# halismai/photobundle

Hardware: AMD Instinct MI355X
Metric: LM iters/sec + residuals/sec, 8-frame KITTI window, 50k pts, 5x5 patch (higher is better)
Workload: dtype f64; 1 GPU; configs[1]: 8-frame window, 50000 points/GPU, 5x5 patch, single level, dense visibility; image=1241x376 u8, observations=400000, sampler_precision=exact, channels=1, point_parameterisation=free world points (reference)

## Files before the change

### photobundle_amd/csrc/pba_batch.h

```cpp
#pragma once
#include "pba_kernels.h"

namespace pba {

constexpr int kMaxBatch = 64;
constexpr int kBatchSampleWaves = 4;

struct BatchWindow {
  SchurParams schur[2];
  ReduceSolveParams rsolve[2];
  SampleParams sample[2];
  const float* frames_mc;
  int32_t channels;
};

struct BatchLaunch {
  const BatchWindow* tab;
  int32_t n;
  int32_t begin[kMaxBatch + 1];
  uint8_t win[kMaxBatch];
  uint8_t mode[kMaxBatch];
  unsigned long long seq[kMaxBatch];
};

__device__ __forceinline__ int batch_entry(const BatchLaunch& L, const int b) {
  int lo = 0, hi = L.n;
  while (hi - lo > 1) {
    const int mid = (lo + hi) >> 1;
    if (L.begin[mid] <= b) lo = mid; else hi = mid;
  }
  return lo;
}

__global__ __launch_bounds__(kTile, 2) void k_schur_batch(const BatchLaunch L) {
  const int k = batch_entry(L, (int)blockIdx.x);
  const int b0 = L.begin[k], lb = (int)blockIdx.x - b0, lgrid = L.begin[k + 1] - b0;
  const int mode = L.mode[k];
  SchurParams p = L.tab[L.win[k]].schur[mode & 1];
  p.init_scale = (mode >> 1) & 1;
  p.pub_seq = L.seq[k] - 1;
  if (!schur_prologue(p, false, lb, (int)threadIdx.x)) return;
  __shared__ __attribute__((aligned(16))) char smem[kSchurSmemBytes];
  schur_body<const void>(p, smem, (int)threadIdx.x, lb, lgrid, nullptr, nullptr, true);
}

__global__ __launch_bounds__(kReduceThreads) void k_reduce_solve_batch(const BatchLaunch L) {
  extern __shared__ __attribute__((aligned(16))) char dyn_smem[];
  const int k = batch_entry(L, (int)blockIdx.x);
  const int b0 = L.begin[k], lb = (int)blockIdx.x - b0, lgrid = L.begin[k + 1] - b0;
  const int mode = L.mode[k];
  ReduceSolveParams rsp = L.tab[L.win[k]].rsolve[mode & 1];
  rsp.so.init_scale = (mode >> 1) & 1;
  if (mode & 1) rsp.fin.seq = L.seq[k];
  reduce_solve_wg(rsp, dyn_smem, lb, lgrid, (int)threadIdx.x);
}

template <int R, bool UNITW>
__global__ __launch_bounds__(kBatchSampleWaves * 64) __attribute__((amdgpu_waves_per_eu((R <= 2 ? PBA_SAMPLE_WAVES_PER_SIMD : (R >= 4 ? PBA_SAMPLE_WAVES_LARGE : 2)), (R <= 2 ? PBA_SAMPLE_WAVES_PER_SIMD : (R >= 4 ? PBA_SAMPLE_WAVES_LARGE : 2)))))
void k_sample_batch(const BatchLaunch L) {
  const int k = batch_entry(L, (int)blockIdx.x);
  const int b0 = L.begin[k], lb = (int)blockIdx.x - b0, lgrid = L.begin[k + 1] - b0;
  const int mode = L.mode[k];
  SampleParams p = L.tab[L.win[k]].sample[mode & 1];
  if (mode & 1) p.seq = L.seq[k];
  if (!sample_prologue<true>(p, false, lb, (int)threadIdx.x)) return;
  __shared__ SampleSmem<R, kBatchSampleWaves> sm;
  ResLane<R> unused;
  sample_wg<R, true, kBatchSampleWaves, true, UNITW, false, false, kMaxFrames, true>(p, sm, unused, xcd_logical_block(lb, lgrid), lgrid, (int)threadIdx.x);
}

template <int R, bool UNITW>
__global__ __launch_bounds__(kBatchSampleWaves * 64) __attribute__((amdgpu_waves_per_eu(PBA_MC_WAVES(R), PBA_MC_WAVES(R)))) void k_sample_mc_batch(const BatchLaunch L) {
  const int k = batch_entry(L, (int)blockIdx.x);
  const int b0 = L.begin[k], lb = (int)blockIdx.x - b0, lgrid = L.begin[k + 1] - b0;
  const int mode = L.mode[k];
  const BatchWindow& bw = L.tab[L.win[k]];
  SampleParams p = bw.sample[mode & 1];
  if (mode & 1) p.seq = L.seq[k];
  if (!sample_prologue<true>(p, false, lb, (int)threadIdx.x)) return;
  sample_mc_wg<R, true, kBatchSampleWaves, true, UNITW>(p, bw.frames_mc, bw.channels, lb, lgrid, (int)threadIdx.x);
}

}
```

### photobundle_amd/csrc/pba_kernels.h

```cpp
#pragma once
#include "pba_device.h"

#include <cfloat>
#include <climits>
#include <type_traits>

#ifndef PBA_PHASE_TIMING
#define PBA_PHASE_TIMING 0
#endif

#ifndef PBA_SAMPLE_WAVES_PER_SIMD
#define PBA_SAMPLE_WAVES_PER_SIMD 4
#endif
#ifndef PBA_SAMPLE_WAVES_LARGE
#define PBA_SAMPLE_WAVES_LARGE 2
#endif
#ifndef PBA_EXPERIMENT_SKIP_IRREGULAR
#define PBA_EXPERIMENT_SKIP_IRREGULAR 0
#endif
#ifndef PBA_WALK_ROWWISE
#define PBA_WALK_ROWWISE 0
#endif

#ifndef PBA_REC_SC1
// ... 469 lines not shown
  if (JAC) {
    sgx = 0.5f * vlerp_exact(dy, omdy, hlerp_exact(dx, omdx, tex_gx2(t11), tex_gx2(t12)), hlerp_exact(dx, omdx, tex_gx2(t21), tex_gx2(t22)));
    sgy = 0.5f * vlerp_exact(dy, omdy, hlerp_exact(dx, omdx, tex_gy2(t11), tex_gy2(t12)), hlerp_exact(dx, omdx, tex_gy2(t21), tex_gy2(t22)));
  }
}

__global__ void k_sample_probe(const uint32_t* __restrict__ frame, int rows, int cols, int n, const float* __restrict__ y,
                               const float* __restrict__ x, float* __restrict__ out) {
  const int i = blockIdx.x * blockDim.x + threadIdx.x;
  if (i >= n) return;
  float sI, sgx, sgy;
  sample_generic<true>(frame, rows, cols, y[i], x[i], sI, sgx, sgy);
  out[3 * i] = sI; out[3 * i + 1] = sgx; out[3 * i + 2] = sgy;
}

struct SampleParams {
  const uint32_t* frames;
  const CamGeom* geom;
  const double* xyz;
  const double* rays;
  const float* desc;
  const double* w2;
  const int32_t* obs_point;
  const uint8_t* obs_slot;
  double* rec;
  double* block_cost;
  int32_t* block_fail;
  int64_t rec_stride;
  int32_t n_obs, n_frames;
  int32_t rows, cols;
  double fx, fy, cx, cy;
  double huber;
  const int4* tile_info;
  const int2* lane_rec;
  const CamGeom* geom_prev;
  const double* xyz_prev;
  const double* rec_prev;
  const double* sp;
  const double* ptrec;
  const double* delta_c;
  double* block_bs;
  unsigned int* ticket;
  unsigned long long* stamp;
  double* scal;
  double* host_scal;
  unsigned long long* host_seq;
  unsigned long long seq;
  int32_t n_tiles;
  int32_t skip_backsub;
  LmState* lm;
  LmState* host_state;
  pba_iteration_summary* log;
  int32_t max_log;
  int32_t enq_cur;
  double* block_cost_alt;
  int32_t* block_fail_alt;
  int32_t decide;
  int32_t prec;
  double* xchg;
  int32_t xchg_rank, xchg_world;
  int32_t xchg_sys;
  unsigned long long* xchg_flag;
  unsigned long long xchg_seq;
  unsigned long long* dbg;
  LmState* lm_init_dst; const LmState* lm_init_src;
  unsigned long long* res_tag; unsigned res_epoch;
};

__device__ __forceinline__ void store_tagged(unsigned long long* w, unsigned ep, double v) {
  const unsigned long long e = (unsigned long long)ep << 32;
  __hip_atomic_store(w, e | (unsigned)__double2hiint(v), __ATOMIC_RELAXED, __HIP_MEMORY_SCOPE_AGENT);
  __hip_atomic_store(w + 1, e | (unsigned)__double2loint(v), __ATOMIC_RELAXED, __HIP_MEMORY_SCOPE_AGENT);
}
__device__ __forceinline__ bool load_tagged(const unsigned long long* w, unsigned ep, double& v) {
  const unsigned long long a = __hip_atomic_load(w, __ATOMIC_RELAXED, __HIP_MEMORY_SCOPE_AGENT);
  const unsigned long long b = __hip_atomic_load(w + 1, __ATOMIC_RELAXED, __HIP_MEMORY_SCOPE_AGENT);
  v = __hiloint2double((int)(unsigned)a, (int)(unsigned)b);
  return (unsigned)(a >> 32) == ep && (unsigned)(b >> 32) == ep;
}

constexpr int kBk = 26;
static_assert(kBk * sizeof(double) <= sizeof(CamGeom), "the compact table fits the second camera-table slot");

__device__ __forceinline__ bool fused_resolve_parity(SampleParams& p) {
  if (p.lm) {
    if (p.lm->done) return false;
    if (p.lm->cur != p.enq_cur) {
      const double* tx = p.xyz; p.xyz = p.xyz_prev; p.xyz_prev = tx;
      double* tr = p.rec; p.rec = const_cast<double*>(p.rec_prev); p.rec_prev = tr;
      const CamGeom* tg = p.geom; p.geom = p.geom_prev; p.geom_prev = tg;
      double* tc = p.block_cost; p.block_cost = p.block_cost_alt; p.block_cost_alt = tc;
      int32_t* tf = p.block_fail; p.block_fail = p.block_fail_alt; p.block_fail_alt = tf;
    }
  }
  return true;
}

template <bool FUSED>
__device__ __forceinline__ bool sample_prologue(SampleParams& p, const bool keep_dbg, const int bid, const int tix) {
  if (!keep_dbg) p.dbg = nullptr;
  if (FUSED && !fused_resolve_parity(p)) return false;
  if (FUSED && p.lm_init_dst && bid == 0 && tix < (int)(sizeof(LmState) / 4))
    reinterpret_cast<unsigned*>(p.lm_init_dst)[tix] = __hip_atomic_load(reinterpret_cast<const unsigned*>(p.lm_init_src) + tix, __ATOMIC_RELAXED, __HIP_MEMORY_SCOPE_SYSTEM);
  return true;
}

struct FusedIdx { int4 ti; int pt, slot, l0, cnt; };
template <int NT>
__device__ __forceinline__ FusedIdx fused_prefetch_indices(const SampleParams& p, int bid, const int tix) {
  FusedIdx f{make_int4(0, 0, 0, 0), 0, 0, 0, 0};
  const int tile = bid * (NT / 128) + (int)(tix >> 7);
  const int lt = tix & 127;
  if (tile < p.n_tiles) {
    f.ti = p.tile_info[tile];
    const int2 r = p.lane_rec[(size_t)tile * 128 + lt];
    f.pt = r.x;
    f.slot = r.y & 0xff; f.l0 = (r.y >> 8) & 0xff; f.cnt = (r.y >> 16) & 0xff;
  }
  return f;
}

template <int NT, bool AG = false>
__device__ __forceinline__ void fused_stage_step_table(const SampleParams& p, double* s_bk, const int tix) {
  if (!p.skip_backsub) {
    constexpr int GW = (int)(sizeof(CamGeom) / 8);
    constexpr int oT = (int)(offsetof(CamGeom, t) / 8), oR = (int)(offsetof(CamGeom, R) / 8), oD = (int)(offsetof(CamGeom, dR) / 8);
    constexpr int oF = (int)(offsetof(CamGeom, free_index) / 4);
    static_assert(offsetof(CamGeom, t) % 8 == 0 && offsetof(CamGeom, R) % 8 == 0 && offsetof(CamGeom, dR) % 8 == 0, "double words");
    const double* G = reinterpret_cast<const double*>(p.geom_prev);
    constexpr int IT = (kBk * kMaxFrames + NT - 1) / NT;
    const int n_e = kBk * p.n_frames;
#pragma unroll
    for (int u = 0; u < IT; ++u) {
      const int e_raw = tix + u * NT;
      const int e = e_raw < n_e ? e_raw : 0;
      const int a = e / kBk, k = e - a * kBk;
      const double* g = G + (size_t)a * GW;
      const double* dc = p.delta_c + 6 * a;
      const bool rot = (k >= 12) && (k < 21);
      const int j = rot ? k - 12 : 0;
      const int o0 = (k < 9) ? oR + k : ((k < 12) ? oT + (k - 9) : oD + j);
      auto ld = [](const double* q) { return AG ? load_agent(q) : *q; };
      const double w0 = ld(g + o0), w1 = ld(g + oD + 9 + j), w2 = ld(g + oD + 18 + j);
      const double d0 = ld(dc), d1 = ld(dc + 1), d2 = ld(dc + 2);
      const double dt = ld(dc + ((k >= 21 && k < 24) ? 3 + (k - 21) : 3));
      const int32_t fidx = AG ? __hip_atomic_load(reinterpret_cast<const int32_t*>(g) + oF, __ATOMIC_RELAXED, __HIP_MEMORY_SCOPE_AGENT)
                              : reinterpret_cast<const int32_t*>(g)[oF];
      double val = rot ? d0 * w0 + d1 * w1 + d2 * w2 : w0;
      if (k >= 21) val = (k < 24) ? dt : (double)fidx;
      if (e_raw < n_e) s_bk[e] = val;
    }
  }
}

template <int NT, class RL = const void>
__device__ __forceinline__ void fused_backsub(const SampleParams& p, const double* rays, const FusedIdx& fi, const double* s_bk,
                                              double* s_bs, int& pt, int& slot, int& obs, bool& active, double (&X)[3],
                                              double& bs_mcc, double& bs_st2, double& bs_x2, const int tix, RL* rl = nullptr) {
  constexpr bool RES = !std::is_void<RL>::value;
  const int half = tix >> 7, lt = tix & 127;
  const int4 ti = fi.ti;
  active = lt < ti.y;
  obs = ti.x + lt;
  int l0 = 0, cnt = 0;
  double c3[3] = {0.0, 0.0, 0.0};
  double pr[12], spk[3] = {1.0, 1.0, 1.0};
// ... 1166 lines not shown
    if (p.huber > 0.0 && cc > p.huber * p.huber) {
      const double r = sqrt(cc);
      rho0 = 2.0 * p.huber * r - p.huber * p.huber;
      rho1 = fmax(DBL_MIN, p.huber / r);
    }
    cost_obs = 0.5 * rho0;
    if (!isfinite(cc)) atomicOr(&s_fail, 1);
    if (JAC) {
      p.rec[0 * p.rec_stride + obs] = rho1 * m11;
      p.rec[1 * p.rec_stride + obs] = rho1 * m12;
      p.rec[2 * p.rec_stride + obs] = rho1 * m22;
      p.rec[3 * p.rec_stride + obs] = rho1 * b1;
      p.rec[4 * p.rec_stride + obs] = rho1 * b2;
      p.rec[5 * p.rec_stride + obs] = cost_obs;
    }
  }
  if (FUSED) {
    lds_barrier();
    fused_wave_step_sums(bs_mcc, bs_st2, bs_x2);
    fused_block_partials<WAVES>(p, bid, lane, wave, cost_obs, bs_mcc, bs_st2, bs_x2, s_red, s_fail, tix);
    fused_finalize<WAVES>(p, lane, wave, &s_base[0][0], reinterpret_cast<double*>(s_raw), 0ull, tix, n_blocks);
  } else {
    const double ws = wave_sum(cost_obs);
    if (lane == 0) s_red[wave] = ws;
    lds_barrier();
    if (tix == 0) {
      double a = 0.0;
#pragma unroll
      for (int w = 0; w < WAVES; ++w) a += s_red[w];
      p.block_cost[bid] = a;
      p.block_fail[bid] = s_fail;
    }
  }
}

template <int R, bool JAC, int WAVES, bool FUSED, bool UNITW, int MF = kMaxFrames>
__global__ __launch_bounds__(WAVES * 64) __attribute__((amdgpu_waves_per_eu(PBA_MC_WAVES(R), PBA_MC_WAVES(R)))) void k_sample_mc(SampleParams p_in, const float* __restrict__ frames_mc, int n_channels) {
  SampleParams p = p_in;
  if (!sample_prologue<FUSED>(p, false, (int)blockIdx.x, (int)threadIdx.x)) return;
  sample_mc_wg<R, JAC, WAVES, FUSED, UNITW, MF>(p, frames_mc, n_channels, (int)blockIdx.x, (int)gridDim.x, (int)threadIdx.x);
}

constexpr int kTile = 128;
constexpr int kObsStride = 37;

constexpr size_t kSchurSmemBytes = sizeof(double) * (kTile * kObsStride + kTile) + kTile * kMaxFrames;

struct SchurParams {
  const double* xyz;
  const double* rays;
  const CamGeom* geom;
  const double* rec;
  const int32_t* obs_point;
  const uint8_t* obs_slot;
  const int4* tile_info;
  const int2* lane_rec;
  double* sp;
  double* ptrec;
  double* partial;
  int64_t rec_stride;
  int32_t n_tiles, n_frames;
  int32_t n_free;
  int32_t n_pairs;
  int32_t part_stride;
  int32_t init_scale;
  int32_t jacobi;
  double fx, fy;
  double radius, inv_radius, min_diag, max_diag;
  unsigned long long* dbg;
  const LmState* lm;
  int32_t enq_cur;
  int32_t final_pass;
  const double* xyz_alt; const CamGeom* geom_alt; const double* rec_alt;
  LmState* pub_state; const double* pub_scal; double* pub_host_scal;
  unsigned long long* pub_host_seq; unsigned long long pub_seq;
  unsigned long long* stamp;
};

__device__ __forceinline__ int sym6(int i, int j) {
  const int a = i < j ? i : j, b = i < j ? j : i;
  return a * 6 - (a * (a - 1)) / 2 + (b - a);
}

template <class RL>
__device__ __forceinline__ void schur_body(SchurParams& p, char* smem, const int tid, const int part, const int n_parts, RL* rl,
                                           const CamGeom* geom_res, const bool has_tile) {
  constexpr bool RES = !std::is_void<RL>::value;
  double* s_obs = reinterpret_cast<double*>(smem);
  static_assert(1024 + kTile * 9 <= kTile * kObsStride && kMaxFrames * sizeof(CamGeom) <= 1024 * sizeof(double), "aliasing fits");
  double* s_vg = s_obs + 1024;
  double* s_tot = s_obs + 1024 + kTile * 9;
  uint16_t* s_ptl = reinterpret_cast<uint16_t*>(s_obs + 1024 + 2 * kTile * 9);
  static_assert(1024 + 2 * kTile * 9 + kTile / 4 <= kTile * kObsStride, "point totals fit before W | Y");
  double* s_red = s_obs + kTile * kObsStride;
  int8_t* s_lane_of = reinterpret_cast<int8_t*>(s_red + kTile);

  const int nf = p.n_free;
  const int n_groups = kTile / p.n_pairs;
  const int grp = tid / p.n_pairs;
  const int pair = tid - grp * p.n_pairs;
  const bool owner = grp < n_groups;
  int pa = 0, pb = 0;
  {
    int a = 0, rem = pair;
    while (rem >= nf - a) { rem -= nf - a; ++a; }
    pa = a; pb = a + rem;
  }
  double acc[36];
#pragma unroll
  for (int k = 0; k < 36; ++k) acc[k] = 0.0;
  constexpr int kCamVals = 33;
  constexpr int kCamAcc = (kCamVals * (kMaxFrames - 1) + kTile - 1) / kTile;
  double acc_cam[kCamAcc];
#pragma unroll
  for (int u = 0; u < kCamAcc; ++u) acc_cam[u] = 0.0;
  double gmax = 0.0, gn2 = 0.0;
  int fail = 0;
  static_assert(sizeof(CamGeom) % 8 == 0, "CamGeom is copied as 8-byte words");
  constexpr int kGeomRegs = 4;
  const int n_geom_words = p.n_frames * (int)(sizeof(CamGeom) / 8);
  unsigned long long greg[kGeomRegs];
#pragma unroll
  for (int u = 0; u < kGeomRegs; ++u) {
    const int k = tid + u * kTile;
    greg[u] = (!RES && k < n_geom_words) ? reinterpret_cast<const unsigned long long*>(p.geom)[k] : 0ull;
  }

  if (tid < kCamVals) s_red[tid] = 0.0;
  static_assert(kCamVals <= kTile, "zero row fits s_red");
  unsigned long long tph[8] = {0, 0, 0, 0, 0, 0, 0, 0};
  unsigned long long tlast = p.dbg ? __builtin_amdgcn_s_memtime() : 0;
  const unsigned long long t_rt0 = p.dbg ? __builtin_amdgcn_s_memrealtime() : 0;
#define PBA_TICK(k) do { if (p.dbg) { const unsigned long long tn = __builtin_amdgcn_s_memtime(); tph[k] += tn - tlast; tlast = tn; } } while (0)
  int4 ti_next = make_int4(0, 0, 0, 0);
  int nx_pt = 0, nx_slot = 0, nx_l0 = 0, nx_cnt = 0;
  double nx_x[3] = {0.0, 0.0, 0.0};
  if constexpr (RES) {
    if (has_tile) { ti_next = rl->ti; nx_pt = rl->pt; nx_slot = rl->slot; nx_l0 = rl->l0; nx_cnt = rl->cnt; nx_x[0] = rl->X[0]; nx_x[1] = rl->X[1]; nx_x[2] = rl->X[2]; }
  } else {
    ti_next = p.tile_info[min(part, p.n_tiles - 1)];
    {
      const int2 r = p.lane_rec[(size_t)min(part, p.n_tiles - 1) * kTile + tid];
      nx_pt = r.x; nx_slot = r.y & 0xff; nx_l0 = (r.y >> 8) & 0xff; nx_cnt = (r.y >> 16) & 0xff;
    }
    if (tid < ti_next.y) {
      nx_x[0] = p.xyz[3 * (size_t)nx_pt]; nx_x[1] = p.xyz[3 * (size_t)nx_pt + 1]; nx_x[2] = p.xyz[3 * (size_t)nx_pt + 2];
    }
  }
  for (int tile = part; RES ? (tile == part) : (tile < p.n_tiles); tile += n_parts) {
    const int4 ti = ti_next;
    if constexpr (!RES) ti_next = p.tile_info[min(tile + n_parts, p.n_tiles - 1)];
    const int cur_pt = nx_pt, cur_slot = nx_slot, cur_l0 = nx_l0, cur_cnt = nx_cnt;
    const double cur_x[3] = {nx_x[0], nx_x[1], nx_x[2]};
    const int o0 = ti.x, n_here = ti.y, pt0 = ti.z, n_pts = ti.w;
    const bool active = tid < n_here;
    const int obs = o0 + tid;

    for (int k = tid; k < kMaxFrames * kTile / 4; k += kTile) reinterpret_cast<uint32_t*>(s_lane_of)[k] = 0x80808080u;
    const CamGeom* s_geom = RES ? geom_res : reinterpret_cast<const CamGeom*>(s_obs);
    if constexpr (!RES) {
#pragma unroll
    for (int u = 0; u < kGeomRegs; ++u) {
      const int k = tid + u * kTile;
      if (k < n_geom_words) reinterpret_cast<unsigned long long*>(s_obs)[k] = greg[u];
    }
    }
    if constexpr (!RES) {
      constexpr int kTail = (kMaxFrames * (int)(sizeof(CamGeom) / 8) + kTile - 1) / kTile - kGeomRegs;
      unsigned long long gt[kTail];
#pragma unroll
      for (int u = 0; u < kTail; ++u) {
        const int k = tid + (kGeomRegs + u) * kTile;
        gt[u] = (k < n_geom_words) ? reinterpret_cast<const unsigned long long*>(p.geom)[k] : 0ull;
      }
#pragma unroll
      for (int u = 0; u < kTail; ++u) {
        const int k = tid + (kGeomRegs + u) * kTile;
        if (k < n_geom_words) reinterpret_cast<unsigned long long*>(s_obs)[k] = gt[u];
      }
    }
    lds_barrier();
    PBA_TICK(0);

    int pt = 0, fa = -1, l0 = 0, l1 = 0;
    double Ac[2][6], Ap[2][3], M[3] = {0, 0, 0}, b[2] = {0, 0};
    double MAp[2][3];
    double s_pt[3] = {1.0, 1.0, 1.0};
    if (active) {
      pt = cur_pt;
      const int slot = cur_slot;
      l0 = cur_l0; l1 = l0 + cur_cnt;
      if constexpr (RES) { if (!p.init_scale) { s_pt[0] = rl->sp[0]; s_pt[1] = rl->sp[1]; s_pt[2] = rl->sp[2]; } }
      else if (!p.init_scale) { s_pt[0] = p.sp[3 * (size_t)pt]; s_pt[1] = p.sp[3 * (size_t)pt + 1]; s_pt[2] = p.sp[3 * (size_t)pt + 2]; }
      const CamGeom& g = s_geom[slot];
      fa = g.free_index;
      const double prm[3] = {cur_x[0], cur_x[1], cur_x[2]};
      double X[3], qd[3];
      point_world(p.rays, pt, prm, X, qd);
      double xw[3];
      transform_point(g, X, xw);
      projection_jacobians(g, X, xw, p.fx, p.fy, Ac, Ap);
      point_jacobian(p.rays, qd, Ap);
      if constexpr (RES) { M[0] = rl->rec[0]; M[1] = rl->rec[1]; M[2] = rl->rec[2]; b[0] = rl->rec[3]; b[1] = rl->rec[4]; }
      else {
      M[0] = p.rec[0 * p.rec_stride + obs]; M[1] = p.rec[1 * p.rec_stride + obs]; M[2] = p.rec[2 * p.rec_stride + obs];
      b[0] = p.rec[3 * p.rec_stride + obs]; b[1] = p.rec[4 * p.rec_stride + obs];
      }
#pragma unroll
      for (int k = 0; k < 3; ++k) { MAp[0][k] = M[0] * Ap[0][k] + M[1] * Ap[1][k]; MAp[1][k] = M[1] * Ap[0][k] + M[2] * Ap[1][k]; }
      double* vg = s_vg + tid * 9;
      vg[0] = Ap[0][0] * MAp[0][0] + Ap[1][0] * MAp[1][0];
      vg[1] = Ap[0][0] * MAp[0][1] + Ap[1][0] * MAp[1][1];
      vg[2] = Ap[0][0] * MAp[0][2] + Ap[1][0] * MAp[1][2];
      vg[3] = Ap[0][1] * MAp[0][1] + Ap[1][1] * MAp[1][1];
      vg[4] = Ap[0][1] * MAp[0][2] + Ap[1][1] * MAp[1][2];
      vg[5] = Ap[0][2] * MAp[0][2] + Ap[1][2] * MAp[1][2];
#pragma unroll
      for (int k = 0; k < 3; ++k) vg[6 + k] = -(Ap[0][k] * b[0] + Ap[1][k] * b[1]);
      if (fa >= 0) s_lane_of[fa * kTile + (pt - pt0)] = (int8_t)tid;
      if (tid == l0) s_ptl[pt - pt0] = (uint16_t)(l0 | ((l1 - l0) << 8));
    }
    lds_barrier();
    PBA_TICK(1);

    double V[6] = {0, 0, 0, 0, 0, 0}, gp[3] = {0, 0, 0};
    for (int k = tid; k < 9 * n_pts; k += kTile) {
      const int q = k / 9, c = k - 9 * q;
      const unsigned lc = s_ptl[q];
      const int ql0 = (int)(lc & 0xffu), qcnt = (int)(lc >> 8);
      const double* src = s_vg + ql0 * 9 + c;
      double a = 0.0;
      double x[8];
#pragma unroll
      for (int l = 0; l < 8; ++l) x[l] = src[9 * (l < qcnt ? l : qcnt - 1)];
#pragma unroll
      for (int l = 0; l < 8; ++l) a += (l < qcnt) ? x[l] : 0.0;
      if (qcnt > 8) {
#pragma unroll
        for (int l = 8; l < kMaxFrames; ++l) x[l - 8] = src[9 * (l < qcnt ? l : qcnt - 1)];
#pragma unroll
        for (int l = 8; l < kMaxFrames; ++l) a += (l < qcnt) ? x[l - 8] : 0.0;
      }
      s_tot[k] = a;
    }
    lds_barrier();
    if (active) {
      const double* tot = s_tot + (pt - pt0) * 9;
#pragma unroll
      for (int k = 0; k < 6; ++k) V[k] = tot[k];
#pragma unroll
      for (int k = 0; k < 3; ++k) gp[k] = tot[6 + k];
    }
    lds_barrier();
    PBA_TICK(2);
    const bool grad_only = p.final_pass != 0 && !p.init_scale;
    double Pm[6] = {0, 0, 0, 0, 0, 0};
    if (active && grad_only) {
      if (tid == l0) {
#pragma unroll
        for (int k = 0; k < 3; ++k) { gmax = fmax(gmax, fabs(gp[k])); gn2 += gp[k] * gp[k]; }
      }
    } else if (active) {
      const bool head = (tid == l0);
      double s[3];
      const double vd[3] = {V[0], V[3], V[5]};
      if (p.init_scale) {
#pragma unroll
        for (int k = 0; k < 3; ++k) s[k] = p.jacobi ? 1.0 / (1.0 + sqrt(vd[k])) : 1.0;
        if constexpr (RES) { rl->sp[0] = s[0]; rl->sp[1] = s[1]; rl->sp[2] = s[2]; }
        else if (head) { p.sp[3 * (size_t)pt] = s[0]; p.sp[3 * (size_t)pt + 1] = s[1]; p.sp[3 * (size_t)pt + 2] = s[2]; }
      } else {
#pragma unroll
        for (int k = 0; k < 3; ++k) s[k] = s_pt[k];
      }
      double D2[3];
#pragma unroll
      for (int k = 0; k < 3; ++k) D2[k] = fmin(fmax(s[k] * s[k] * vd[k], p.min_diag), p.max_diag) * p.inv_radius;
      const double a00 = s[0] * s[0] * V[0] + D2[0], a01 = s[0] * s[1] * V[1], a02 = s[0] * s[2] * V[2];
      const double a11 = s[1] * s[1] * V[3] + D2[1], a12 = s[1] * s[2] * V[4], a22 = s[2] * s[2] * V[5] + D2[2];
      bool pd = a00 > 0.0;
      const double i00 = fast_rsqrt(a00);
      const double l10 = a01 * i00, l20 = a02 * i00;
      const double d1 = a11 - l10 * l10;
      pd = pd && d1 > 0.0;
      const double i11 = fast_rsqrt(d1);
      const double l21 = (a12 - l20 * l10) * i11;
      const double d2 = a22 - l20 * l20 - l21 * l21;
      pd = pd && d2 > 0.0;
      const double i22 = fast_rsqrt(d2);
      if (pd) {
        const double i10 = -l10 * i00 * i11;
        const double i21 = -l21 * i11 * i22;
        const double i20 = -(l20 * i00 + l21 * i10) * i22;
        const double v00 = i00 * i00 + i10 * i10 + i20 * i20;
        const double v01 = i10 * i11 + i20 * i21;
        const double v02 = i20 * i22;
        const double v11 = i11 * i11 + i21 * i21;
        const double v12 = i21 * i22;
        const double v22 = i22 * i22;
        Pm[0] = s[0] * s[0] * v00; Pm[1] = s[0] * s[1] * v01; Pm[2] = s[0] * s[2] * v02;
        Pm[3] = s[1] * s[1] * v11; Pm[4] = s[1] * s[2] * v12; Pm[5] = s[2] * s[2] * v22;
      } else if (head) {
        fail = 1;
      }
      if constexpr (RES) {
#pragma unroll
        for (int k = 0; k < 6; ++k) rl->pr[k] = Pm[k];
#pragma unroll
        for (int k = 0; k < 3; ++k) { rl->pr[6 + k] = gp[k]; rl->pr[9 + k] = D2[k]; }
      }
// ... 164 lines not shown
  } else {
    if (owner && grp > 0) {
      double* dst = s_obs + ((grp - 1) * p.n_pairs + pair) * 36;
#pragma unroll
      for (int k = 0; k < 36; ++k) dst[k] = acc[k];
    }
    lds_barrier();
    if (owner && grp == 0) {
      for (int g = 1; g < n_groups; ++g) {
        const double* src = s_obs + ((g - 1) * p.n_pairs + pair) * 36;
#pragma unroll
        for (int k = 0; k < 36; ++k) acc[k] += src[k];
      }
    }
  }
  lds_barrier();
  PBA_TEP(1);
  const int n = 6 * nf;
  double* s_cam = spread ? s_obs + n_ent : s_obs;
#pragma unroll
  for (int u = 0; u < kCamAcc; ++u) {
    const int e = tid + u * kTile;
    if (e < kCamVals * nf) {
      s_cam[e] = acc_cam[u];
      const int a = e / kCamVals, v = e - a * kCamVals;
      if (v >= 27) put(out_at(36 * p.n_pairs + n + 6 * a + (v - 27)), acc_cam[u], false);
      else if (v >= 21) put(out_at(36 * p.n_pairs + 6 * a + (v - 21)), acc_cam[u], false);
      else {
#pragma unroll
        for (int i = 0; i < 6; ++i) if (v == 6 * i - (i * (i - 1)) / 2) put(out_at(36 * p.n_pairs + 2 * n + 6 * a + i), acc_cam[u], false);
      }
    }
  }
  lds_barrier();
  PBA_TEP(2);
  if (spread) {
#pragma unroll 1
    for (int e = tid; e < n_ent; e += kTile) {
      const int k = e / p.n_pairs, pe = e - k * p.n_pairs;
      int a = 0, rem = pe;
      while (rem >= nf - a) { rem -= nf - a; ++a; }
      double v = s_obs[e];
      if (rem == 0) { const int i = k / 6, j = k - 6 * i; v += s_cam[a * kCamVals + sym6(i, j)]; }
      put(out_at(PBA_PARTIAL_T ? e : pe * 36 + k), v, PBA_PARTIAL_SC1 != 0);
    }
  } else if (owner && grp == 0) {
    if (pa == pb) {
      const double* U = s_cam + pa * kCamVals;
#pragma unroll
      for (int i = 0; i < 6; ++i)
#pragma unroll
        for (int j = 0; j < 6; ++j) acc[6 * i + j] += U[sym6(i, j)];
    }
#pragma unroll
    for (int k = 0; k < 36; ++k) {
      put(out_at(PBA_PARTIAL_T ? k * p.n_pairs + pair : pair * 36 + k), acc[k], PBA_PARTIAL_SC1 != 0);
    }
  }
  lds_barrier();
  PBA_TEP(3);
  {
    const double g2 = wave_sum(gn2), gm = wave_max(gmax), fl = wave_max((double)fail);
    if ((tid & 63) == 0) { s_red[(tid >> 6) * 3] = g2; s_red[(tid >> 6) * 3 + 1] = gm; s_red[(tid >> 6) * 3 + 2] = fl; }
    lds_barrier();
    if (tid == 0) {
      double a = 0.0, m = 0.0, f = 0.0;
      for (int w = 0; w < kTile / 64; ++w) { a += s_red[3 * w]; m = fmax(m, s_red[3 * w + 1]); f = fmax(f, s_red[3 * w + 2]); }
      put(out_at(36 * p.n_pairs + 3 * n + 0), m, false);
      put(out_at(36 * p.n_pairs + 3 * n + 1), a, false);
      put(out_at(36 * p.n_pairs + 3 * n + 2), f, false);
      if (!RES && p.stamp && part < kStampSchurBlocks) p.stamp[kStampSchur0 + part] = __builtin_amdgcn_s_memrealtime();
    }
  }
  PBA_TEP(4);
  if (RES && p.dbg && tid == 0) for (int k = 0; k < 4; ++k) p.dbg[part * 16 + 8 + k] = tep[k + 1] - tep[k];
#undef PBA_TEP
}

__device__ __forceinline__ bool schur_prologue(SchurParams& p, const bool keep_dbg, const int bid, const int tix) {
  if (!keep_dbg) p.dbg = nullptr;
  if (p.pub_host_seq && bid == 0)
    lm_publish(p.lm, p.pub_state, p.pub_scal, p.pub_host_scal, p.pub_host_seq, p.pub_seq, tix, kTile);
  if (p.lm) {
    if (p.lm->done && !p.final_pass) return false;
    if (p.final_pass && !lm_final_pass_needed(p.lm)) return false;
    if (p.lm->cur != p.enq_cur) { p.xyz = p.xyz_alt; p.geom = p.geom_alt; p.rec = p.rec_alt; }
    p.radius = p.lm->radius;
    p.inv_radius = 1.0 / p.radius;
  }
  return true;
}

__global__ __launch_bounds__(kTile, 2) void k_schur(SchurParams p_in) {
  SchurParams p = p_in;
  if (!schur_prologue(p, PBA_PHASE_TIMING != 0, (int)blockIdx.x, (int)threadIdx.x)) return;
  __shared__ __attribute__((aligned(16))) char smem[kSchurSmemBytes];
  schur_body<const void>(p, smem, (int)threadIdx.x, (int)blockIdx.x, (int)gridDim.x, nullptr, nullptr, true);
}

}

#include "pba_solve.h"

namespace pba {

struct BacksubParams {
  const double* xyz;
  const double* rays;
  double* xyz_cand;
  const CamGeom* geom;
  const double* rec;
  const int32_t* pt_begin;
  const uint8_t* obs_slot;
  const double* sp;
  const double* ptrec;
  const double* delta_c;
  double* block_out;
  const double* cams_cand;
  CamGeom* geom_cand;
  int64_t rec_stride;
  int32_t n_points, n_frames;
  uint32_t anchor_mask;
  double fx, fy;
};

__global__ __launch_bounds__(256) void k_backsub(BacksubParams p) {
  __shared__ double s_red[3][256];
  const int tid = threadIdx.x;
  const int pt = blockIdx.x * 256 + tid;
  if (p.geom_cand && blockIdx.x == gridDim.x - 1 && tid >= 256 - p.n_frames) cam_geom_one(p.cams_cand, p.geom_cand, 255 - tid, p.anchor_mask);
  double mcc = 0.0, st2 = 0.0, x2 = 0.0;
  if (pt < p.n_points) {
    const double X[3] = {p.xyz[3 * (size_t)pt], p.xyz[3 * (size_t)pt + 1], p.xyz[3 * (size_t)pt + 2]};
    double Xw[3], qd[3];
    point_world(p.rays, pt, X, Xw, qd);
    double acc[3] = {0, 0, 0};
    for (int o = p.pt_begin[pt]; o < p.pt_begin[pt + 1]; ++o) {
      const int slot = p.obs_slot[o];
      const CamGeom& g = p.geom[slot];
      if (g.free_index < 0) continue;
      double xw[3], Ac[2][6], Ap[2][3];
      transform_point(g, Xw, xw);
      projection_jacobians(g, Xw, xw, p.fx, p.fy, Ac, Ap);
      point_jacobian(p.rays, qd, Ap);
      const double* dc = p.delta_c + 6 * slot;
      double t0 = 0.0, t1 = 0.0;
#pragma unroll
      for (int k = 0; k < 6; ++k) { t0 += Ac[0][k] * dc[k]; t1 += Ac[1][k] * dc[k]; }
      const double m0 = p.rec[0 * p.rec_stride + o], m1 = p.rec[1 * p.rec_stride + o], m2 = p.rec[2 * p.rec_stride + o];
      const double u0 = m0 * t0 + m1 * t1, u1 = m1 * t0 + m2 * t1;
#pragma unroll
      for (int k = 0; k < 3; ++k) acc[k] += Ap[0][k] * u0 + Ap[1][k] * u1;
    }
    const double* pr = p.ptrec + 12 * (size_t)pt;
    const double q0 = pr[6] + acc[0], q1 = pr[7] + acc[1], q2 = pr[8] + acc[2];
    const double d0 = -(pr[0] * q0 + pr[1] * q1 + pr[2] * q2);
    const double d1 = -(pr[1] * q0 + pr[3] * q1 + pr[4] * q2);
    const double d2 = -(pr[2] * q0 + pr[4] * q1 + pr[5] * q2);
    const double d[3] = {d0, d1, d2};
#pragma unroll
    for (int k = 0; k < 3; ++k) {
      const double s = p.sp[3 * (size_t)pt + k];
      const double yk = -d[k] / s;
      mcc += 0.5 * yk * (s * pr[6 + k]) + 0.5 * pr[9 + k] * yk * yk;
      st2 += d[k] * d[k];
      x2 += X[k] * X[k];
      p.xyz_cand[3 * (size_t)pt + k] = X[k] + d[k];
    }
  }
  s_red[0][tid] = mcc; s_red[1][tid] = st2; s_red[2][tid] = x2;
  __syncthreads();
  for (int s = 128; s > 0; s >>= 1) {
    if (tid < s) { s_red[0][tid] += s_red[0][tid + s]; s_red[1][tid] += s_red[1][tid + s]; s_red[2][tid] += s_red[2][tid + s]; }
    __syncthreads();
  }
  if (tid == 0) { p.block_out[3 * blockIdx.x] = s_red[0][0]; p.block_out[3 * blockIdx.x + 1] = s_red[1][0]; p.block_out[3 * blockIdx.x + 2] = s_red[2][0]; }
}

__global__ __launch_bounds__(256) void k_finalize_step(const double* __restrict__ bs_out, int n_bs_blocks,
                                                        const double* __restrict__ block_cost,
// ... 48 lines not shown
```

### photobundle_amd/csrc/pba_solve.h

```cpp
#pragma once

namespace pba {

__host__ __device__ inline int tri_index(int r) { return r * (r + 1) / 2; }
__host__ __device__ inline int packed_stride(int n) { return tri_index(n + 1) + 2 * n + 2; }

__host__ __device__ inline int solve_item_base(int j, int N1) { return (j - 1) * (N1 - 3 * j); }
inline int solve_table_words(int nf) { const int n = 6 * nf; return tri_index(n + 1) + (nf > 1 ? solve_item_base(nf, n + 1) : 0); }
inline void solve_tables(int nf, uint32_t* tab) {
  const int n = 6 * nf, N1 = n + 1, TRI = tri_index(N1);
  for (int r = 0; r < N1; ++r)
    for (int c = 0; c <= r; ++c) tab[tri_index(r) + c] = ((uint32_t)r << 16) | (uint32_t)c;
  for (int j = 1; j < nf; ++j)
    for (int r = 6 * j; r <= n; ++r) tab[TRI + solve_item_base(j, N1) + (r - 6 * j)] = (uint32_t)r | ((uint32_t)j << 16);
}

__device__ __forceinline__ int packed_dest(int e, int nf, int n_pairs) {
  const int n = 6 * nf, nT = 36 * n_pairs;
  if (e < nT) {
    const int pair = PBA_PARTIAL_T ? e % n_pairs : e / 36, k = PBA_PARTIAL_T ? e / n_pairs : e - 36 * pair, i = k / 6, j = k - 6 * i;
    int a = 0, rem = pair;
    while (rem >= nf - a) { rem -= nf - a; ++a; }
    const int b = a + rem;
    if (a == b && j < i) return -1;
// ... 56 lines not shown
      acc[r] = 0.0;
      if (valid) {
#pragma unroll
        for (int k = 0; k < NF; ++k) acc[r] = is_max ? fmax(acc[r], v[r][k]) : acc[r] + v[r][k];
        for (int b = sub + NF * SUB; b < n_blocks; b += NF * SUB) {
#pragma unroll
          for (int k = 0; k < NF; ++k) {
            const int bb = b + SUB * k;
            v[r][k] = (bb < n_blocks) ? ldp(rp.partial + ((size_t)vb * n_blocks + bb) * EX + ex) : 0.0;
          }
#pragma unroll
          for (int k = 0; k < NF; ++k) acc[r] = is_max ? fmax(acc[r], v[r][k]) : acc[r] + v[r][k];
        }
      }
      static_assert(EX == 16, "lane = 16 (sub % 4) + ex");
#pragma unroll
      for (int off = 16; off <= 32; off <<= 1) {
        const double o = __shfl_xor(acc[r], off);
        acc[r] = is_max ? fmax(acc[r], o) : acc[r] + o;
      }
      if ((tid & 63) < EX) s_red[(tid + r * T) >> 6][ex] = acc[r];
    }
    __syncthreads();
    if (tid < EX && valid) {
      double s = s_red[0][ex];
#pragma unroll
      for (int w = 1; w < kReduceThreads / 64; ++w) s = is_max ? fmax(s, s_red[w][ex]) : s + s_red[w][ex];
      if (dest >= 0) packed_store<STORE>(rp.packed + dest, s);
      else if (e == stride - 3) packed_store<STORE>(rp.scal + kGmaxPts, s);
      else if (e == stride - 2) packed_store<STORE>(rp.packed + TRI + 2 * n + 1, s);
      else if (e == stride - 1) packed_store<STORE>(rp.scal + kSchurFail, s);
    }
  } else {
#pragma unroll
    for (int r = 0; r < ROLES; ++r) {
      double acc = 0.0; int f = 0;
      for (int b = tid + r * T; b < rp.n_cost_blocks; b += kReduceThreads) {
        acc += ldp(rp.block_cost + b);
        f |= AGL ? __hip_atomic_load(rp.block_fail + b, __ATOMIC_RELAXED, __HIP_MEMORY_SCOPE_AGENT) : rp.block_fail[b];
      }
      acc = wave_sum(acc);
      f = __any(f) ? 1 : 0;
      if ((tid & 63) == 0) { s_red[(tid + r * T) >> 6][0] = acc; s_f[(tid + r * T) >> 6] = f; }
    }
    __syncthreads();
    if (tid == 0) {
      double s = s_red[0][0]; int ff = s_f[0];
      for (int w = 1; w < kReduceThreads / 64; ++w) { s += s_red[w][0]; ff |= s_f[w]; }
      packed_store<STORE>(rp.packed + TRI + 2 * n, s);
      packed_store<STORE>(rp.scal + kEvalFailLin, (double)ff);
      if (n >= 0) packed_store<STORE>(rp.packed + tri_index(n) + n, 0.0);
    }
  }
}

struct SolveParams {
  const double* packed;
  const double* cams;
  double* cams_cand;
  double* delta_c;
  double* sc;
  double* S_dbg;
  double* rhs_dbg;
  double* scal;
  const CamGeom* geom;
  CamGeom* geom_cand;
  const uint32_t* tab;
  int32_t n_frames, n_free, n_pairs, stride;
  uint32_t anchor_mask;
  int32_t init_scale, jacobi;
  double radius, min_diag, max_diag;
  const LmState* lm;
  int32_t enq_cur, final_pass;
  int32_t dbg;
  const double* cams_alt; double* cams_cand_alt; const CamGeom* geom_alt; CamGeom* geom_cand_alt;
  PeerParams peer;
  int32_t peer_world, peer_flag;
  unsigned long long peer_off, peer_seq, peer_timeout;
  unsigned int* peer_err;
};

__device__ __forceinline__ bool solve_resolve(SolveParams& p) {
  if (!p.lm) return true;
  if (p.lm->done && !p.final_pass) return false;
  if (p.final_pass && !lm_final_pass_needed(p.lm)) return false;
  if (p.lm->cur != p.enq_cur) {
    p.cams = p.cams_alt; p.cams_cand = p.cams_cand_alt; p.geom = p.geom_alt;
    if (p.geom_cand) p.geom_cand = p.geom_cand_alt;
  }
  p.radius = p.lm->radius;
  return true;
}

__device__ __forceinline__ void tri_row_col(int t, int& r, int& c) {
  r = (int)((sqrtf(8.0f * (float)t + 1.0f) - 1.0f) * 0.5f);
  while (tri_index(r + 1) <= t) ++r;
  while (tri_index(r) > t) --r;
  c = t - tri_index(r);
}

template <bool AGENT>
__device__ __forceinline__ double packed_load(const SolveParams& p, int idx) {
  if (AGENT) return load_agent(p.packed + idx);
  if (p.peer_world > 0) return peer_sum(p.peer, p.peer_world, p.peer_off, idx);
  return p.packed[idx];
}

constexpr int kSolveThreads = 256;

template <int T>
__device__ __forceinline__ void solve_prologue(const SolveParams& p, int n, int ld, double* S, double* y, double* sc,
                                               double* D2, double* gcs, double* gc, int tid) {
  const int TRI = tri_index(n + 1);
  for (int i = tid; i < n; i += T) {
    const double du = packed_load<false>(p, TRI + n + i);
    const double g = packed_load<false>(p, TRI + i);
    double s;
    if (p.init_scale) { s = p.jacobi ? 1.0 / (1.0 + sqrt(du)) : 1.0; p.sc[i] = s; p.sc[n + i] = du > 0.0 ? 1.0 : 0.0; }
    else s = p.sc[i];
    sc[i] = s;
    D2[i] = fmin(fmax(s * s * du, p.min_diag), p.max_diag) / p.radius;
    gc[i] = g;
    gcs[i] = s * g;
  }
  __syncthreads();
  for (int t = tid; t < TRI - 1; t += T) {
    int r, c;
    tri_row_col(t, r, c);
    const double val = packed_load<false>(p, t);
    if (r == n) { y[c] = sc[c] * val; continue; }
    double v = sc[c] * val * sc[r];
    if (r == c) v += D2[r];
    S[r * ld + c] = v;
    S[c * ld + r] = v;
  }
  __syncthreads();
  if (p.S_dbg) {
    for (int k = tid; k < n * n; k += T) p.S_dbg[k] = S[(k / n) * ld + (k % n)];
    for (int i = tid; i < n; i += T) p.rhs_dbg[i] = y[i];
  }
  __syncthreads();
}

template <int T>
__device__ __forceinline__ void solve_epilogue(const SolveParams& p, int n, const double* y, const double* sc,
                                               const double* D2, const double* gcs, const double* gc, bool chol_ok,
                                               int tid) {
  if (tid < 6 * p.n_frames && !(p.final_pass && !p.init_scale)) {
    const int slot = tid / 6, k = tid % 6;
    const int fa = p.geom[slot].free_index;
    double d = 0.0;
    if (fa >= 0) d = -sc[6 * fa + k] * y[6 * fa + k];
    p.delta_c[tid] = d;
    p.cams_cand[tid] = p.cams[tid] + d;
  }
  if (p.geom_cand) {
    const int c = tid - (T - 64);
    if (c >= 0 && c < p.n_frames) {
      double cam6[6];
      const int fa = p.geom[c].free_index;
      for (int k = 0; k < 6; ++k) cam6[k] = p.cams[6 * c + k] + (fa >= 0 ? -sc[6 * fa + k] * y[6 * fa + k] : 0.0);
      cam_geom_one(cam6 - 6 * c, p.geom_cand, c, p.anchor_mask);
    }
  }
  if (tid < 64) {
    double mcc = 0.0, st2 = 0.0, x2 = 0.0, gmax = 0.0, gn2 = 0.0, bad = 0.0;
    for (int i = tid; i < n; i += 64) {
      mcc += 0.5 * y[i] * gcs[i] + 0.5 * D2[i] * y[i] * y[i];
      const double d = sc[i] * y[i];
      st2 += d * d;
      gmax = fmax(gmax, fabs(gc[i]));
      gn2 += gc[i] * gc[i];
      if (!isfinite(y[i])) bad = 1.0;
// ... 473 lines not shown
    p.scal[kMccCams] = s_dyn[0]; p.scal[kStep2Cams] = s_dyn[1]; p.scal[kX2Cams] = s_stat[2];
    p.scal[kGmaxCams] = s_stat[0]; p.scal[kGnorm2Cams] = s_stat[1];
    p.scal[kSolveOk] = (chol_ok && s_dyn[2] == 0.0 && !poisoned) ? 1.0 : 0.0;
    p.scal[kCostLin] = poisoned ? qnan : cost_lin;
    p.scal[kGnorm2Pts] = gn2_pts;
  }
  PBA_TS(6);
  if (p.geom_cand) {
    __syncthreads();
    for (int c = tid / 32; c < p.n_frames; c += T / 32) cam_geom_finish(s_cg[c], p.geom_cand, c, p.anchor_mask, tid & 31);
  }
  PBA_TS(5);
  if (PBA_PHASE_TIMING && p.dbg && tid == 0)
    printf("solve_blocked n %d cycles: prologue %llu (loads + tables %llu, scatter %llu) factorisation %llu [block %llu rows %llu Lb %llu barrier %llu update %llu reload %llu] substitution %llu epilogue %llu (scalars %llu)\n",
           n, ts[2] - ts[0], ts[1] - ts[0], ts[2] - ts[1], ts[3] - ts[2], sec[1], sec[2], sec[3], sec[4], sec[5], sec[6], ts[4] - ts[3], ts[5] - ts[4], ts[6] - ts[4]);
#undef PBA_TS
#undef PBA_SEC
}

template <int T>
__global__ __launch_bounds__(T) void k_solve_blocked(SolveParams p_in) {
  SolveParams p = p_in;
  if (!solve_resolve(p)) return;
  extern __shared__ __attribute__((aligned(16))) char smem[];
  solve_blocked<false, T>(p, reinterpret_cast<double*>(smem), threadIdx.x);
}

struct ReduceFinalParams {
  ReduceParams rp;
  const LmState* lm; int32_t enq_cur, final_pass;
  const double* block_cost_alt; const int32_t* block_fail_alt;
  int32_t sys_stores;
  unsigned int* ticket;
  double* peer_own; int32_t peer_flag; unsigned long long peer_seq;
};
__global__ __launch_bounds__(kReduceThreads) void k_reduce_final(ReduceFinalParams fp) {
  ReduceParams rp = fp.rp;
  const bool skip = fp.lm && ((fp.lm->done && !fp.final_pass) || (fp.final_pass && !lm_final_pass_needed(fp.lm)));
  __shared__ double s_red[kReduceThreads / kReduceEntries][kReduceEntries + 1];
  __shared__ int s_f[16];
  if (!skip) {
    if (fp.lm && fp.lm->cur != fp.enq_cur) { rp.block_cost = fp.block_cost_alt; rp.block_fail = fp.block_fail_alt; }
    if (fp.sys_stores) reduce_partials<2>(rp, s_red, s_f, (int)blockIdx.x, (int)gridDim.x);
    else reduce_partials<0>(rp, s_red, s_f, (int)blockIdx.x, (int)gridDim.x);
  }
  if (fp.peer_flag >= 0) {
    asm volatile("s_waitcnt vmcnt(0)" ::: "memory");
    __syncthreads();
    if (threadIdx.x == 0) {
      const unsigned t = __hip_atomic_fetch_add(fp.ticket, 1u, __ATOMIC_ACQ_REL, __HIP_MEMORY_SCOPE_AGENT);
      if (t == gridDim.x - 1) {
        *fp.ticket = 0;
        __hip_atomic_store(reinterpret_cast<unsigned long long*>(fp.peer_own) + fp.peer_flag, fp.peer_seq, __ATOMIC_RELEASE, __HIP_MEMORY_SCOPE_SYSTEM);
      }
    }
  }
}

struct ReduceSolveParams {
  ReduceParams rp;
  const double* block_cost_alt; const int32_t* block_fail_alt;
  unsigned int* ticket;
  unsigned long long* stamp;
  SolveParams so;
  struct Fin {
    LmState* lm; pba_iteration_summary* log; pba_iteration_summary* host_log; int32_t max_log;
    LmState* host_state; double* host_scal; unsigned long long* host_seq; unsigned long long seq;
  } fin;
};

__device__ inline void flush_to_host(const LmState* lm, LmState* host_state, const double* scal, double* host_scal, const pba_iteration_summary* log,
                                     pba_iteration_summary* host_log, int max_log, unsigned long long* host_seq, unsigned long long seq, int tid, int nthreads) {
  const int n_words = (lm->n_log < max_log ? lm->n_log : max_log) * (int)(sizeof(pba_iteration_summary) / 4);
  static_assert(sizeof(pba_iteration_summary) % 4 == 0, "word copy");
  const unsigned* src = reinterpret_cast<const unsigned*>(log);
  for (int k = tid; k < n_words; k += nthreads) store_system_u32(reinterpret_cast<unsigned*>(host_log) + k, src[k]);
  lm_publish(lm, host_state, scal, host_scal, host_seq, seq, tid, nthreads);
}

__device__ __forceinline__ void reduce_solve_wg(const ReduceSolveParams rsp, char* dyn_smem, const int bid, const int grid, const int tid) {
  const LmState* lm = rsp.so.lm;
  ReduceParams rp = rsp.rp;
  const bool fin_mode = rsp.fin.host_seq != nullptr;
  if (lm) {
    if (lm->done && !rsp.so.final_pass) return;
    if (rsp.so.final_pass && !lm_final_pass_needed(lm)) {
      if (fin_mode && bid == 0)
        flush_to_host(lm, rsp.fin.host_state, rsp.so.scal, rsp.fin.host_scal, rsp.fin.log, rsp.fin.host_log, rsp.fin.max_log, rsp.fin.host_seq,
                      rsp.fin.seq, tid, kReduceThreads);
      return;
    }
    if (lm->cur != rsp.so.enq_cur) { rp.block_cost = rsp.block_cost_alt; rp.block_fail = rsp.block_fail_alt; }
  }
  const unsigned long long t_k0 = PBA_PHASE_TIMING ? __builtin_amdgcn_s_memrealtime() : 0ull;
  __shared__ double s_red[kReduceThreads / kReduceEntries][kReduceEntries + 1];
  __shared__ int s_f[16];
  __shared__ int s_last;
  reduce_partials<1>(rp, s_red, s_f, bid, grid);
  asm volatile("s_waitcnt vmcnt(0)" ::: "memory");
  __syncthreads();
  if (tid == 0) {
    const unsigned t = __hip_atomic_fetch_add(rsp.ticket, 1u, __ATOMIC_RELAXED, __HIP_MEMORY_SCOPE_AGENT);
    s_last = (t == (unsigned)grid - 1) ? 1 : 0;
  }
  __syncthreads();
  if (!s_last) return;
  const bool wide = rsp.so.n_free > kSolveNarrowFree;
  static_assert(kSolveWideThreads == kReduceThreads, "the wide solve uses the whole workgroup");
  if (!wide && tid >= kSolveBlockedThreads) return;
  if (tid == 0) *rsp.ticket = 0;
  const unsigned long long t_k1 = PBA_PHASE_TIMING ? __builtin_amdgcn_s_memrealtime() : 0ull;
  SolveParams so = rsp.so;
  if (so.lm) {
    if (so.lm->cur != so.enq_cur) {
      so.cams = so.cams_alt; so.cams_cand = so.cams_cand_alt; so.geom = so.geom_alt;
      if (so.geom_cand) so.geom_cand = so.geom_cand_alt;
    }
    so.radius = so.lm->radius;
  }
  so.packed = rp.packed;
  if (wide) solve_blocked<true, kSolveWideThreads>(so, reinterpret_cast<double*>(dyn_smem), tid);
  else solve_blocked<true, kSolveBlockedThreads>(so, reinterpret_cast<double*>(dyn_smem), tid);
  if (fin_mode) {
    const int nth = wide ? kSolveWideThreads : kSolveBlockedThreads;
    __syncthreads();
    if (tid == 0) {
      double sl[kNumScal];
      for (int k = 0; k < kNumScal; ++k) sl[k] = load_agent(so.scal + k);
      lm_decide(rsp.fin.lm, sl, rsp.fin.log, rsp.fin.max_log, 1);
      if (rsp.fin.lm->done && rsp.fin.lm->done_seq == 0) rsp.fin.lm->done_seq = rsp.fin.seq;
    }
    __syncthreads();
    __builtin_amdgcn_fence(__ATOMIC_ACQUIRE, "agent");
    flush_to_host(rsp.fin.lm, rsp.fin.host_state, so.scal, rsp.fin.host_scal, rsp.fin.log, rsp.fin.host_log, rsp.fin.max_log, rsp.fin.host_seq,
                  rsp.fin.seq, tid, nth);
  }
  if (rsp.stamp && tid == 0) rsp.stamp[kStampEndSolve] = __builtin_amdgcn_s_memrealtime();
  if (PBA_PHASE_TIMING && rsp.so.dbg && tid == 0)
    printf("k_reduce_solve: last workgroup %d of %d reached the solve %.2f us after its own start, finished it %.2f us later\n", bid,
           grid, 0.01 * (double)(t_k1 - t_k0), 0.01 * (double)(__builtin_amdgcn_s_memrealtime() - t_k1));
}

__global__ __launch_bounds__(kReduceThreads) void k_reduce_solve(ReduceSolveParams rsp) {
  extern __shared__ __attribute__((aligned(16))) char dyn_smem[];
  reduce_solve_wg(rsp, dyn_smem, (int)blockIdx.x, (int)gridDim.x, (int)threadIdx.x);
}

}
```

Baseline: 9848 LM iters/s of the one 50000-point window (50k points per GPU: weak scaling; not multiplied by N).

## Prefetch Schur tile head and per-obs records early; skip Hessian gather on b-only pass

Issues the first tile's info and lane-record loads before the LM-state prologue so their latency overlaps the prologue. Hoists the per-observation rec and scale loads to the top of each tile. Loads the LM head fields once into scalar registers, and reuses the reduce kernel's cur and radius reads in the solve. On the final gradient-only pass the V-block accumulation is skipped. This adds register pressure and relies on the head read staying consistent across the prologue.

```diff
diff --git a/photobundle_amd/csrc/pba_batch.h b/photobundle_amd/csrc/pba_batch.h
--- a/photobundle_amd/csrc/pba_batch.h
+++ b/photobundle_amd/csrc/pba_batch.h
@@ -39,9 +39,10 @@
   SchurParams p = L.tab[L.win[k]].schur[mode & 1];
   p.init_scale = (mode >> 1) & 1;
   p.pub_seq = L.seq[k] - 1;
+  const SchurHead head = schur_prefetch_head(p, lb, (int)threadIdx.x);
   if (!schur_prologue(p, false, lb, (int)threadIdx.x)) return;
   __shared__ __attribute__((aligned(16))) char smem[kSchurSmemBytes];
-  schur_body<const void>(p, smem, (int)threadIdx.x, lb, lgrid, nullptr, nullptr, true);
+  schur_body<const void>(p, smem, (int)threadIdx.x, lb, lgrid, nullptr, nullptr, true, &head);
 }
 
 __global__ __launch_bounds__(kReduceThreads) void k_reduce_solve_batch(const BatchLaunch L) {
diff --git a/photobundle_amd/csrc/pba_kernels.h b/photobundle_amd/csrc/pba_kernels.h
--- a/photobundle_amd/csrc/pba_kernels.h
+++ b/photobundle_amd/csrc/pba_kernels.h
@@ -575,6 +575,18 @@
 constexpr int kBk = 26;
 static_assert(kBk * sizeof(double) <= sizeof(CamGeom), "the compact table fits the second camera-table slot");
 
+struct LmHead { int32_t done, cur; double radius; };
+__device__ __forceinline__ LmHead lm_load_head(const LmState* lm) {
+  int32_t d = lm->done, c = lm->cur;
+  double r = lm->radius;
+  asm volatile("" : "+v"(d), "+v"(c), "+v"(r));
+  LmHead h;
+  h.done = __builtin_amdgcn_readfirstlane(d);
+  h.cur = __builtin_amdgcn_readfirstlane(c);
+  h.radius = __hiloint2double(__builtin_amdgcn_readfirstlane(__double2hiint(r)), __builtin_amdgcn_readfirstlane(__double2loint(r)));
+  return h;
+}
+
 __device__ __forceinline__ bool fused_resolve_parity(SampleParams& p) {
   if (p.lm) {
     if (p.lm->done) return false;
@@ -1907,9 +1919,18 @@
   return a * 6 - (a * (a - 1)) / 2 + (b - a);
 }
 
+struct SchurHead { int4 ti; int2 lr; };
+__device__ __forceinline__ SchurHead schur_prefetch_head(const SchurParams& p, const int part, const int tid) {
+  SchurHead h;
+  const int t0 = min(part, p.n_tiles - 1);
+  h.ti = p.tile_info[t0];
+  h.lr = p.lane_rec[(size_t)t0 * kTile + tid];
+  return h;
+}
+
 template <class RL>
 __device__ __forceinline__ void schur_body(SchurParams& p, char* smem, const int tid, const int part, const int n_parts, RL* rl,
-                                           const CamGeom* geom_res, const bool has_tile) {
+                                           const CamGeom* geom_res, const bool has_tile, const SchurHead* head = nullptr) {
   constexpr bool RES = !std::is_void<RL>::value;
   double* s_obs = reinterpret_cast<double*>(smem);
   static_assert(1024 + kTile * 9 <= kTile * kObsStride && kMaxFrames * sizeof(CamGeom) <= 1024 * sizeof(double), "aliasing fits");
@@ -1963,9 +1984,9 @@
   if constexpr (RES) {
     if (has_tile) { ti_next = rl->ti; nx_pt = rl->pt; nx_slot = rl->slot; nx_l0 = rl->l0; nx_cnt = rl->cnt; nx_x[0] = rl->X[0]; nx_x[1] = rl->X[1]; nx_x[2] = rl->X[2]; }
   } else {
-    ti_next = p.tile_info[min(part, p.n_tiles - 1)];
+    ti_next = head->ti;
     {
-      const int2 r = p.lane_rec[(size_t)min(part, p.n_tiles - 1) * kTile + tid];
+      const int2 r = head->lr;
       nx_pt = r.x; nx_slot = r.y & 0xff; nx_l0 = (r.y >> 8) & 0xff; nx_cnt = (r.y >> 16) & 0xff;
     }
     if (tid < ti_next.y) {
@@ -1980,6 +2001,15 @@
     const int o0 = ti.x, n_here = ti.y, pt0 = ti.z, n_pts = ti.w;
     const bool active = tid < n_here;
     const int obs = o0 + tid;
+    const bool b_only = !RES && p.final_pass != 0 && !p.init_scale;
+    double ld_rec[5] = {0.0, 0.0, 0.0, 0.0, 0.0}, ld_sp[3] = {1.0, 1.0, 1.0};
+    if constexpr (!RES) {
+      if (active) {
+        if (!b_only) { ld_rec[0] = p.rec[0 * p.rec_stride + obs]; ld_rec[1] = p.rec[1 * p.rec_stride + obs]; ld_rec[2] = p.rec[2 * p.rec_stride + obs]; }
+        ld_rec[3] = p.rec[3 * p.rec_stride + obs]; ld_rec[4] = p.rec[4 * p.rec_stride + obs];
+        if (!p.init_scale) { ld_sp[0] = p.sp[3 * (size_t)cur_pt]; ld_sp[1] = p.sp[3 * (size_t)cur_pt + 1]; ld_sp[2] = p.sp[3 * (size_t)cur_pt + 2]; }
+      }
+    }
 
     for (int k = tid; k < kMaxFrames * kTile / 4; k += kTile) reinterpret_cast<uint32_t*>(s_lane_of)[k] = 0x80808080u;
     const CamGeom* s_geom = RES ? geom_res : reinterpret_cast<const CamGeom*>(s_obs);
@@ -2016,7 +2046,7 @@
       const int slot = cur_slot;
       l0 = cur_l0; l1 = l0 + cur_cnt;
       if constexpr (RES) { if (!p.init_scale) { s_pt[0] = rl->sp[0]; s_pt[1] = rl->sp[1]; s_pt[2] = rl->sp[2]; } }
-      else if (!p.init_scale) { s_pt[0] = p.sp[3 * (size_t)pt]; s_pt[1] = p.sp[3 * (size_t)pt + 1]; s_pt[2] = p.sp[3 * (size_t)pt + 2]; }
+      else { s_pt[0] = ld_sp[0]; s_pt[1] = ld_sp[1]; s_pt[2] = ld_sp[2]; }
       const CamGeom& g = s_geom[slot];
       fa = g.free_index;
       const double prm[3] = {cur_x[0], cur_x[1], cur_x[2]};
@@ -2027,10 +2057,7 @@
       projection_jacobians(g, X, xw, p.fx, p.fy, Ac, Ap);
       point_jacobian(p.rays, qd, Ap);
       if constexpr (RES) { M[0] = rl->rec[0]; M[1] = rl->rec[1]; M[2] = rl->rec[2]; b[0] = rl->rec[3]; b[1] = rl->rec[4]; }
-      else {
-      M[0] = p.rec[0 * p.rec_stride + obs]; M[1] = p.rec[1 * p.rec_stride + obs]; M[2] = p.rec[2 * p.rec_stride + obs];
-      b[0] = p.rec[3 * p.rec_stride + obs]; b[1] = p.rec[4 * p.rec_stride + obs];
-      }
+      else { M[0] = ld_rec[0]; M[1] = ld_rec[1]; M[2] = ld_rec[2]; b[0] = ld_rec[3]; b[1] = ld_rec[4]; }
 #pragma unroll
       for (int k = 0; k < 3; ++k) { MAp[0][k] = M[0] * Ap[0][k] + M[1] * Ap[1][k]; MAp[1][k] = M[1] * Ap[0][k] + M[2] * Ap[1][k]; }
       double* vg = s_vg + tid * 9;
@@ -2051,6 +2078,7 @@
     double V[6] = {0, 0, 0, 0, 0, 0}, gp[3] = {0, 0, 0};
     for (int k = tid; k < 9 * n_pts; k += kTile) {
       const int q = k / 9, c = k - 9 * q;
+      if (b_only && c < 6) continue;
       const unsigned lc = s_ptl[q];
       const int ql0 = (int)(lc & 0xffu), qcnt = (int)(lc >> 8);
       const double* src = s_vg + ql0 * 9 + c;
@@ -2381,10 +2409,13 @@
   if (p.pub_host_seq && bid == 0)
     lm_publish(p.lm, p.pub_state, p.pub_scal, p.pub_host_scal, p.pub_host_seq, p.pub_seq, tix, kTile);
   if (p.lm) {
-    if (p.lm->done && !p.final_pass) return false;
+    const LmHead h = lm_load_head(p.lm);
+    const int32_t done = h.done, cur = h.cur;
+    const double radius = h.radius;
+    if (done && !p.final_pass) return false;
     if (p.final_pass && !lm_final_pass_needed(p.lm)) return false;
-    if (p.lm->cur != p.enq_cur) { p.xyz = p.xyz_alt; p.geom = p.geom_alt; p.rec = p.rec_alt; }
-    p.radius = p.lm->radius;
+    if (cur != p.enq_cur) { p.xyz = p.xyz_alt; p.geom = p.geom_alt; p.rec = p.rec_alt; }
+    p.radius = radius;
     p.inv_radius = 1.0 / p.radius;
   }
   return true;
@@ -2392,9 +2423,10 @@
 
 __global__ __launch_bounds__(kTile, 2) void k_schur(SchurParams p_in) {
   SchurParams p = p_in;
+  const SchurHead head = schur_prefetch_head(p, (int)blockIdx.x, (int)threadIdx.x);
   if (!schur_prologue(p, PBA_PHASE_TIMING != 0, (int)blockIdx.x, (int)threadIdx.x)) return;
   __shared__ __attribute__((aligned(16))) char smem[kSchurSmemBytes];
-  schur_body<const void>(p, smem, (int)threadIdx.x, (int)blockIdx.x, (int)gridDim.x, nullptr, nullptr, true);
+  schur_body<const void>(p, smem, (int)threadIdx.x, (int)blockIdx.x, (int)gridDim.x, nullptr, nullptr, true, &head);
 }
 
 }
diff --git a/photobundle_amd/csrc/pba_solve.h b/photobundle_amd/csrc/pba_solve.h
--- a/photobundle_amd/csrc/pba_solve.h
+++ b/photobundle_amd/csrc/pba_solve.h
@@ -162,13 +162,16 @@
 
 __device__ __forceinline__ bool solve_resolve(SolveParams& p) {
   if (!p.lm) return true;
-  if (p.lm->done && !p.final_pass) return false;
+  const LmHead h = lm_load_head(p.lm);
+  const int32_t done = h.done, cur = h.cur;
+  const double radius = h.radius;
+  if (done && !p.final_pass) return false;
   if (p.final_pass && !lm_final_pass_needed(p.lm)) return false;
-  if (p.lm->cur != p.enq_cur) {
+  if (cur != p.enq_cur) {
     p.cams = p.cams_alt; p.cams_cand = p.cams_cand_alt; p.geom = p.geom_alt;
     if (p.geom_cand) p.geom_cand = p.geom_cand_alt;
   }
-  p.radius = p.lm->radius;
+  p.radius = radius;
   return true;
 }
 
@@ -808,15 +811,21 @@
   const LmState* lm = rsp.so.lm;
   ReduceParams rp = rsp.rp;
   const bool fin_mode = rsp.fin.host_seq != nullptr;
+  bool alt = false;
+  double radius = rsp.so.radius;
   if (lm) {
-    if (lm->done && !rsp.so.final_pass) return;
+    const LmHead h = lm_load_head(lm);
+    const int32_t done = h.done, cur = h.cur;
+    radius = h.radius;
+    if (done && !rsp.so.final_pass) return;
     if (rsp.so.final_pass && !lm_final_pass_needed(lm)) {
       if (fin_mode && bid == 0)
         flush_to_host(lm, rsp.fin.host_state, rsp.so.scal, rsp.fin.host_scal, rsp.fin.log, rsp.fin.host_log, rsp.fin.max_log, rsp.fin.host_seq,
                       rsp.fin.seq, tid, kReduceThreads);
       return;
     }
-    if (lm->cur != rsp.so.enq_cur) { rp.block_cost = rsp.block_cost_alt; rp.block_fail = rsp.block_fail_alt; }
+    alt = cur != rsp.so.enq_cur;
+    if (alt) { rp.block_cost = rsp.block_cost_alt; rp.block_fail = rsp.block_fail_alt; }
   }
   const unsigned long long t_k0 = PBA_PHASE_TIMING ? __builtin_amdgcn_s_memrealtime() : 0ull;
   __shared__ double s_red[kReduceThreads / kReduceEntries][kReduceEntries + 1];
@@ -837,13 +846,11 @@
   if (tid == 0) *rsp.ticket = 0;
   const unsigned long long t_k1 = PBA_PHASE_TIMING ? __builtin_amdgcn_s_memrealtime() : 0ull;
   SolveParams so = rsp.so;
-  if (so.lm) {
-    if (so.lm->cur != so.enq_cur) {
-      so.cams = so.cams_alt; so.cams_cand = so.cams_cand_alt; so.geom = so.geom_alt;
-      if (so.geom_cand) so.geom_cand = so.geom_cand_alt;
-    }
-    so.radius = so.lm->radius;
-  }
+  if (alt) {
+    so.cams = so.cams_alt; so.cams_cand = so.cams_cand_alt; so.geom = so.geom_alt;
+    if (so.geom_cand) so.geom_cand = so.geom_cand_alt;
+  }
+  so.radius = radius;
   so.packed = rp.packed;
   if (wide) solve_blocked<true, kSolveWideThreads>(so, reinterpret_cast<double*>(dyn_smem), tid);
   else solve_blocked<true, kSolveBlockedThreads>(so, reinterpret_cast<double*>(dyn_smem), tid);
```

Result: faster. 9947 LM iters/s of the one 50000-point window (50k points per GPU: weak scaling; not multiplied by N), median of 4 (+1.0%).
